# youtalk/opencv-ar

Measured on AMD Instinct MI355X. Metric: frames/sec at 1920x1080, 16 markers/frame; 1/2/4/8 MI355X, higher is better.
Workload: dtype u8

## Files before the change

opencv-ar_amd/csrc/follow.hip:

```cpp
#include "kernels.h"
#include "trace_core.h"

namespace ocvar {

__device__ __forceinline__ int ticket_lane() {
    int l = (int)(threadIdx.x & 63);
    asm volatile("" : "+v"(l));
    return l;
}
__device__ __forceinline__ int uni(int v) { return __builtin_amdgcn_readfirstlane(v); }
__device__ __forceinline__ unsigned uni(unsigned v) { return (unsigned)__builtin_amdgcn_readfirstlane((int)v); }
__device__ __forceinline__ unsigned long long uni(unsigned long long v) {
    return ((unsigned long long)uni((unsigned)(v >> 32)) << 32) | uni((unsigned)v);
}
__device__ __forceinline__ double uni(double v) { return __longlong_as_double((long long)uni((unsigned long long)__double_as_longlong(v))); }

#ifdef OCVAR_PROF
#define PROF_NOW() __builtin_readcyclecounter()
#define PROF_DECL() unsigned long long prof_acc[16] = {0, 0, 0, 0, 0, 0, 0, 0, 0, 0, 0, 0, 0, 0, 0, 0}
#define PROF_ADD(slot, v) do { prof_acc[slot] += (unsigned long long)(v); } while (0)
#define PROF_FLUSH(base) do { if ((threadIdx.x & 63) == 0) for (int i_ = 0; i_ < 16; i_++) if (i_ != 7) atomicAdd(reinterpret_cast<unsigned long long*>(ws.counters + CNT_PROF) + (base) + i_, prof_acc[i_]); } while (0)
#else
#define PROF_NOW() 0ull
#define PROF_DECL() do { } while (0)
#define PROF_ADD(slot, v) do { (void)(v); } while (0)
#define PROF_FLUSH(base) do { } while (0)
#endif

constexpr int FW = 1;
constexpr int FOLLOW_THREADS = 64 * FW;

struct PlaneRef {
    const uint8_t* nbr;
    int ns, sh, img_w, img_h, plane;
};

template <bool CROP>
__device__ __forceinline__ PlaneRef plane_of(const Workspace& ws, int roi) {
    PlaneRef p;
    if (CROP) {
        const Roi r = ws.rois_crop[roi];
        p.ns = r.ns; p.sh = r.sh; p.img_w = r.w; p.img_h = r.h;
        p.nbr = ws.nbr_crop + r.nbr_off;
    } else {
        p.ns = ws.ns; p.sh = ws.sh; p.img_w = ws.W; p.img_h = ws.H;
        p.nbr = ws.nbr_frame + (size_t)roi * nbr_plane_bytes(ws.ns, ws.sh);
    }
    p.plane = p.ns * p.sh;
    return p;
}

template <bool CROP>
__device__ __forceinline__ void emit_quad(const Workspace& ws, const StartCand c, const int* dst);

template <bool CROP>
__device__ __forceinline__ void approximate_and_emit(const Workspace& ws, const StartCand c, const PlaneRef& pl, const int* pts,
                                                     int npts, double perimeter, DpSlice* stack, bool emit = true) {
    int dst[2 * (DP_MAX_OUT + 1)];
    const int m = approx_poly_dp(pts, npts, perimeter * 0.02, dst, stack);
    if (m != 4 || !quad_filter(dst, pl.img_w, pl.img_h)) return;
    if (emit) emit_quad<CROP>(ws, c, dst);
}

template <bool CROP>
__device__ __forceinline__ void emit_quad(const Workspace& ws, const StartCand c, const int* dst) {
    QuadRec q;
    q.roi = c.roi;
    q.start = c.pos;
    for (int k = 0; k < 8; k++) q.pt[k] = dst[k];
    if (CROP) {
        const int slot = atomicAdd(ws.counters + CNT_CROP_QUADS, 1);
        if (slot >= ws.cap_crop_quads) {
            atomicOr(ws.counters + CNT_ERR, ERR_QUAD_OVERFLOW);
            return;
        }
        ws.quads_crop[slot] = q;
        atomicMin(ws.best_crop + c.roi, ((unsigned long long)(unsigned)c.pos << 32) | (unsigned)slot);
    } else {
        const int slot = atomicAdd(ws.n_quads_frame + c.roi, 1);
        if (slot >= ws.maxq) {
            atomicOr(ws.counters + CNT_ERR, ERR_QUAD_OVERFLOW);
            return;
        }
        ws.quads_frame[(size_t)c.roi * ws.maxq + slot] = q;
    }
}

template <int CTRL, int ROWS = 0xf>
__device__ __forceinline__ unsigned dpp_self(unsigned v) {
    return (unsigned)__builtin_amdgcn_update_dpp((int)v, (int)v, CTRL, ROWS, 0xf, false);
}
template <int CTRL, int ROWS = 0xf>
__device__ __forceinline__ unsigned dpp_zero(unsigned v) {
    return (unsigned)__builtin_amdgcn_update_dpp(0, (int)v, CTRL, ROWS, 0xf, false);
}
#define OCVAR_WAVE_LADDER(STEP) \
    STEP(0xB1, 0xf) STEP(0x4E, 0xf) STEP(0x141, 0xf) STEP(0x140, 0xf) STEP(0x142, 0xa) STEP(0x143, 0xc)

__device__ __forceinline__ unsigned wave_max_u32(unsigned v) {
#define STEP(C, R) { const unsigned o = dpp_self<C, R>(v); v = o > v ? o : v; }
    OCVAR_WAVE_LADDER(STEP)
#undef STEP
    return (unsigned)__builtin_amdgcn_readlane((int)v, 63);
}
__device__ __forceinline__ unsigned long long wave_max_u64(unsigned long long v) {
#define STEP(C, R) { const unsigned long long o = ((unsigned long long)dpp_self<C, R>((unsigned)(v >> 32)) << 32) | dpp_self<C, R>((unsigned)v); v = o > v ? o : v; }
    OCVAR_WAVE_LADDER(STEP)
#undef STEP
    return ((unsigned long long)(unsigned)__builtin_amdgcn_readlane((int)(unsigned)(v >> 32), 63) << 32) |
           (unsigned)__builtin_amdgcn_readlane((int)(unsigned)v, 63);
}
typedef unsigned short us2v __attribute__((ext_vector_type(2)));
__device__ __forceinline__ unsigned pk_min(unsigned a, unsigned b) { return __builtin_bit_cast(unsigned, __builtin_elementwise_min(__builtin_bit_cast(us2v, a), __builtin_bit_cast(us2v, b))); }
__device__ __forceinline__ unsigned pk_max(unsigned a, unsigned b) { return __builtin_bit_cast(unsigned, __builtin_elementwise_max(__builtin_bit_cast(us2v, a), __builtin_bit_cast(us2v, b))); }
__device__ __forceinline__ unsigned wave_pk_min(unsigned v) {
#define STEP(C, R) v = pk_min(v, dpp_self<C, R>(v));
    OCVAR_WAVE_LADDER(STEP)
#undef STEP
    return (unsigned)__builtin_amdgcn_readlane((int)v, 63);
}
__device__ __forceinline__ unsigned wave_pk_max(unsigned v) {
#define STEP(C, R) v = pk_max(v, dpp_self<C, R>(v));
    OCVAR_WAVE_LADDER(STEP)
#undef STEP
    return (unsigned)__builtin_amdgcn_readlane((int)v, 63);
}
__device__ __forceinline__ double wave_sum_f64(double v) {
#define STEP(C, R) { const unsigned long long b = (unsigned long long)__double_as_longlong(v); \
                     v += __longlong_as_double((long long)(((unsigned long long)dpp_zero<C, R>((unsigned)(b >> 32)) << 32) | dpp_zero<C, R>((unsigned)b))); }
    OCVAR_WAVE_LADDER(STEP)
#undef STEP
    const unsigned long long b = (unsigned long long)__double_as_longlong(v);
    return __longlong_as_double((long long)(((unsigned long long)(unsigned)__builtin_amdgcn_readlane((int)(unsigned)(b >> 32), 63) << 32) |
                                            (unsigned)__builtin_amdgcn_readlane((int)(unsigned)b, 63)));
}

__device__ __forceinline__ int px_of(unsigned p) { return (int)(p & 0xffffu); }
__device__ __forceinline__ int py_of(unsigned p) { return (int)(p >> 16); }

constexpr int LDS_PTS = SLAB_PTS;
constexpr int DP_DST = 2 * (DP_MAX_OUT + 1);

struct WaveScratch {
    DpSlice stack[DP_STACK];
    int dst[DP_DST];
};

template <bool K32>
__device__ __forceinline__ int wave_approx_dp(const unsigned* src, int count, double parameter, int* dst, DpSlice* stack) {
    const int lane = threadIdx.x & 63;
    float eps = (float)parameter;
    eps *= eps;
    int top = 0, new_count = 0;
    DpSlice slice = {0, 0}, right = {0, 0};
    int sx = 0, sy = 0;
    bool le_eps = false;
    int pos = 0;
    for (int it = 0; it < 3; it++) {
        pos = (pos + right.start) % count;
        const unsigned sp = uni(src[pos]);
        sx = px_of(sp);
        sy = py_of(sp);
        int max_dist = 0;
        if (K32) {
            unsigned best = 0;
            for (int j = 1 + lane; j < count; j += 64) {
                int q = pos + j;
// ... 88 lines not shown
        }
        if (le_eps) {
            if (new_count >= DP_MAX_OUT) return DP_MAX_OUT + 1;
            dst[2 * new_count] = sx;
            dst[2 * new_count + 1] = sy;
            new_count++;
        } else {
            right.end = slice.end;
            slice.end = right.start;
            if (new_count + top + 2 > DP_MAX_OUT) return DP_MAX_OUT + 1;
            if (lane == 0) {
                stack[top] = right;
                stack[top + 1] = slice;
            }
            top += 2;
        }
    }
    __builtin_amdgcn_fence(__ATOMIC_ACQ_REL, "workgroup");
    const int n = new_count;
    int r = n - 1;
    sx = dst[2 * r];
    sy = dst[2 * r + 1];
    if (++r >= n) r = 0;
    int wpos = r;
    int px = dst[2 * r], py = dst[2 * r + 1];
    if (++r >= n) r = 0;
    for (int i = 0; i < n && new_count > 2; i++) {
        const int ex = dst[2 * r], ey = dst[2 * r + 1];
        if (++r >= n) r = 0;
        const int dx = ex - sx, dy = ey - sy;
        int dist = (px - sx) * dy - (py - sy) * dx;
        dist = dist < 0 ? -dist : dist;
        if ((double)dist * dist <= 0.5 * eps * (dx * dx + dy * dy) && dx != 0 && dy != 0) {
            new_count--;
            dst[2 * wpos] = sx = ex;
            dst[2 * wpos + 1] = sy = ey;
            if (++wpos >= n) wpos = 0;
            px = dst[2 * r];
            py = dst[2 * r + 1];
            if (++r >= n) r = 0;
            i++;
            continue;
        }
        dst[2 * wpos] = sx = px;
        dst[2 * wpos + 1] = sy = py;
        if (++wpos >= n) wpos = 0;
        px = ex;
        py = ey;
    }
    __builtin_amdgcn_fence(__ATOMIC_ACQ_REL, "workgroup");
    return new_count;
}

template <bool CROP, bool STAGE>
__device__ __forceinline__ bool wave_finish_packed(const Workspace& ws, const StartCand c, const PlaneRef& pl, const unsigned* gsrc, int npts,
                                                   unsigned* lpts, WaveScratch* sc) {
    const int lane = threadIdx.x & 63;
    if (npts < 4) return false;
    unsigned lo = 0xffffffffu, hi = 0u;
    if (STAGE) {
        unsigned v[LDS_PTS / 64];
#pragma unroll
        for (int k = 0; k < LDS_PTS / 64; k++) {
            const int i = lane + 64 * k;
            v[k] = i < npts ? gsrc[i] : 0u;
        }
#pragma unroll
        for (int k = 0; k < LDS_PTS / 64; k++) {
            const int i = lane + 64 * k;
            if (i < npts) {
                lpts[i] = v[k];
                lo = pk_min(lo, v[k]);
                hi = pk_max(hi, v[k]);
            }
        }
    } else {
        for (int i = lane; i < npts; i += 64) {
            const unsigned p = gsrc[i];
            lo = pk_min(lo, p);
            hi = pk_max(hi, p);
        }
    }
    lo = wave_pk_min(lo);
    hi = wave_pk_max(hi);
    const int bw = px_of(hi) - px_of(lo), bh = py_of(hi) - py_of(lo);
    if (!((long long)bw * bh > 500)) return false;
    __builtin_amdgcn_fence(__ATOMIC_ACQ_REL, "workgroup");
    const unsigned* src = STAGE ? lpts : gsrc;
    double per = 0.0;
    for (int i = lane; i < npts; i += 64) {
        const unsigned p = src[i], q = src[i == 0 ? npts - 1 : i - 1];
        const float dx = (float)px_of(p) - (float)px_of(q), dy = (float)py_of(p) - (float)py_of(q);
        per += (double)sqrt_rn(dx * dx + dy * dy);
    }
    per = wave_sum_f64(per);
#ifdef OCVAR_PROF
    if (lane == 0) atomicAdd(reinterpret_cast<unsigned long long*>(ws.counters + CNT_PROF) + (CROP ? 16 : 0) + 7, 1ull);
#endif
    const bool k32 = npts <= 1024 && (long long)bw * bw + (long long)bh * bh < (1ll << 21);
    const int m = k32 ? wave_approx_dp<true>(src, npts, per * 0.02, sc->dst, sc->stack) : wave_approx_dp<false>(src, npts, per * 0.02, sc->dst, sc->stack);
    if (m != 4) return false;
    int q[8];
#pragma unroll
    for (int k = 0; k < 8; k++) q[k] = uni(sc->dst[k]);
    if (!quad_filter(q, pl.img_w, pl.img_h)) return false;
    if (lane == 0) emit_quad<CROP>(ws, c, q);
    return true;
}

template <bool CROP>
__device__ __forceinline__ int follow_short(const Workspace& ws, const StartCand c) {
    const int BUDGET = SHORT_STEPS;
    const PlaneRef pl = plane_of<CROP>(ws, c.roi);
    if (c.pos <= 0 || c.pos >= pl.plane) return false;
    {
        if (earlier_start_behind(pl.nbr, pl.ns, pl.plane, c.pos, c.is_hole, BACK_STEPS)) return 0;
        if (CROP) {
            const int x = c.pos % pl.ns, y = c.pos / pl.ns;
            return (x == 1 || y == 1) ? 3 : 1;
        }
        const LeanTrace lt = trace_flat(pl.nbr, pl.ns, pl.plane, c.pos, c.is_hole, nullptr, 0, BUDGET);
        if (lt.status == TRACE_OVERRUN) return lt.npts <= 2 ? 2 : 1;
        if (lt.status != TRACE_OK || lt.npts < 4) return 0;
        return 1;
    }
    return 0;
}

template <bool CROP>
__device__ int follow_overflow(const Workspace& ws, const StartCand c, const PlaneRef& pl) {
    const TraceStats st = trace_border<false, false>(pl.nbr, pl.ns, pl.plane, c.pos, c.is_hole, nullptr, 0, ws.mid_steps);
    if (st.status == TRACE_OVERRUN) return 1;
    if (!worth_approximating(st)) return 0;
    const int need = 2 * st.npts + 2 * (st.npts + 2);
    const long long off = atomicAdd(reinterpret_cast<unsigned long long*>(ws.counters + CNT_POOL_INTS), (unsigned long long)need);
    if (off + need > ws.cap_pool_ints) {
        atomicOr(ws.counters + CNT_ERR, ERR_POOL_OVERFLOW);
        return 0;
    }
    int* pts = ws.pool + off;
    trace_border<true, false>(pl.nbr, pl.ns, pl.plane, c.pos, c.is_hole, pts, st.npts, ws.mid_steps);
    approximate_and_emit<CROP>(ws, c, pl, pts, st.npts, st.perimeter, reinterpret_cast<DpSlice*>(pts + 2 * st.npts));
    return 0;
}

constexpr int T1_TICKET = 512;
constexpr int T1_OUT = 128;

template <bool CROP>
__global__ __launch_bounds__(FOLLOW_THREADS) void follow_kernel(Workspace ws) {
    const StartCand* cands = CROP ? ws.cands_crop : ws.cands_frame;
    int n = ws.counters[CROP ? CNT_CROP_CANDS : CNT_FRAME_CANDS];
    const int cap = CROP ? ws.cap_crop_cands : ws.cap_frame_cands;
    if (n > cap) n = cap;
    int* ticket = ws.counters + (CROP ? CNT_TICKET_C : CNT_TICKET_F);
    const int lane = threadIdx.x & 63;
    const int wave = uni((int)(threadIdx.x >> 6));
    const unsigned long long below = (1ull << lane) - 1ull;
    __shared__ StartCand wqueue[FW][128];
// ... 129 lines not shown
    const unsigned dx = (unsigned)(step_dx((int)e) + 1), dy = (unsigned)(step_dy((int)e) + 1);
    const unsigned pw = ((12u - from) & 7u) < t, pe = ((8u - from) & 7u) < t;
    return dx | (dy << 16) | (((e + 5u) & 7u) << 5) | (e << 10) | (pe << 30) | (pw << 31);
}

struct LeanWalk {
    unsigned xy;
    unsigned m;
    unsigned from;
    unsigned pe;
    unsigned xy0, xy1;
    unsigned cxy;
    int npts, step, status;
};

__device__ __forceinline__ void lean_begin(LeanWalk& w, const uint8_t* nbr, int ns, int cpos, int is_hole) {
    const int i0 = cpos - is_hole;
    const int x = i0 % ns, y = i0 / ns;
    w.xy = w.xy0 = (unsigned)x | ((unsigned)y << 16);
    w.cxy = w.xy0 + (unsigned)is_hole;
    w.npts = 0;
    w.step = 0;
    w.status = -1;
    w.xy1 = 0;
    w.pe = 0;
    w.from = 0;
    w.m = nbr_of(nbr, x, y, ns);
    if (w.m == 0) {
        w.status = TRACE_SINGLE;
        w.npts = 1;
        return;
    }
    const int s = first_cw(w.m, (is_hole ? 0 : 4) - 1);
    w.xy1 = w.xy0 + (unsigned)(step_dx(s) + 65536 * step_dy(s));
    w.pe = (unsigned)(s ^ 4) << 10;
    w.from = (unsigned)(s + 1) & 7u;
}

template <class Park>
__device__ __forceinline__ void lean_step(LeanWalk& w, const unsigned* tab, const uint8_t* base, unsigned nt, unsigned last, Park&& park) {
    const unsigned mm = __builtin_amdgcn_perm(w.m, w.m, 0u);
    const unsigned t = (unsigned)__builtin_ctz(__builtin_amdgcn_alignbit(mm, mm, w.from));
    const unsigned ent = tab[(t << 3) + w.from];
    const int d = (int)(w.xy - w.cxy);
    const unsigned nf = ((ent << 1) & (unsigned)(d + 1)) | (ent & (unsigned)d);
    const unsigned nxy = w.xy + (ent & LW_DELTA) - 0x10001u;
    const bool closes = (nxy == w.xy0) & (w.xy == w.xy1);
    const unsigned e = ent & LW_EXIT;
    const bool emit = e != w.pe;
    unsigned off = nbr_win_off_xy(nxy, nt);
    off = off < last ? off : last;
    const unsigned* win = reinterpret_cast<const unsigned*>(base + off);
    const unsigned m4 = nbr_mask9(win[0], win[1], win[2], nxy & 15u);
    park(w.xy);
    w.npts += emit ? 1 : 0;
    w.status = (int)nf < 0 ? (int)TRACE_NOT_FIRST : closes ? (int)TRACE_OK : m4 == 0u ? (int)TRACE_OVERRUN : -1;
    w.step += 1;
    w.xy = nxy;
    w.pe = e;
    w.from = (ent >> 5) & 7u;
    w.m = m4;
}

constexpr int MID_BLOCK = 32;
constexpr int POINT_ROW = MID_BLOCK + 1;
constexpr int FLUSH_W = MID_BLOCK <= 16 ? 16 : 32;
static_assert(FLUSH_W >= MID_BLOCK && 64 % FLUSH_W == 0, "a group of lanes covers a whole row of parked points");

template <bool CROP>
__global__ __launch_bounds__(FOLLOW_THREADS) void follow_mid_kernel(Workspace ws, int phase) {
    __shared__ WaveScratch scratch[FW];
    __shared__ unsigned parked[FW][64 * POINT_ROW];
    __shared__ unsigned step_tab[64];
    if (threadIdx.x < 64u) step_tab[threadIdx.x] = lean_table_entry(threadIdx.x);
    __syncthreads();
    const StartCand* cands = CROP ? ws.mid_crop : ws.mid_frame;
    StartCand* longs = CROP ? ws.long_crop : ws.long_frame;
    int n = ws.counters[CROP ? CNT_MID_C : CNT_MID_F];
    if (n > ws.cap_long) n = ws.cap_long;
    int n_first = (CROP && phase != 2) ? ws.counters[CNT_MID_C_FIRST] : 0;
    if (n_first > ws.cap_long) n_first = ws.cap_long;
    n += n_first;
    int* ticket = ws.counters + (CROP ? (phase == 2 ? CNT_TICKET_MC2 : CNT_TICKET_MC) : CNT_TICKET_MF);
    int* n_long = ws.counters + (CROP ? CNT_LONG_C : CNT_LONG_F);
    const int lane = threadIdx.x & 63;
    const int wave = uni((int)(threadIdx.x >> 6));
    const unsigned long long below = (1ull << lane) - 1ull;
    unsigned* wave_slabs = reinterpret_cast<unsigned*>(ws.slab) + ((size_t)blockIdx.x * blockDim.x + uni((int)(threadIdx.x & ~63u))) * SLAB_STRIDE;
    static_assert(64 * POINT_ROW >= LDS_PTS, "the staging area of the approximation aliases the (flushed) point rows");
    unsigned* my_row = parked[wave] + lane * POINT_ROW;
    const unsigned* wave_rows = parked[wave];
    int flushed = 0;
    const int budget = ws.mid_steps;
    bool have = false;
    bool more = true;
    StartCand c;
    c.roi = 0; c.pos = 0; c.is_hole = 0;
    PlaneRef pl = plane_of<CROP>(ws, 0);
    LeanWalk w;
    w.xy = w.m = w.from = w.pe = w.xy0 = w.xy1 = w.cxy = 0u;
    w.npts = w.step = 0;
    w.status = TRACE_NOT_FIRST;
    unsigned pl_nt = 1u, pl_last = 0u;
    long long guard = ((long long)n + 64) * (budget / MID_BLOCK + 5) + 64;
    PROF_DECL();
    for (;;) {
        if (--guard < 0) {
            if (lane == 0) atomicOr(ws.counters + CNT_ERR, ERR_TICKET_RUNAWAY);
            break;
        }
        const unsigned long long pt0 = PROF_NOW();
        for (int tries = 0; tries < (CROP ? 4 : 1); tries++) {
            const unsigned long long idle = __ballot(!have);
            if (!(more && idle)) break;
            if (tries > 0) --guard;
            const int cnt = __popcll(idle);
            int base = 0;
            if (ticket_lane() == 0) base = atomicAdd(ticket, cnt);
            base = uni(base);
            if (base + cnt >= n) more = false;
            if (!have) {
                const int idx = base + __popcll(idle & below);
                if (idx < n) {
                    c = (CROP && idx < n_first) ? ws.mid_first_crop[idx] : cands[idx - n_first];
                    bool take = true;
                    if (CROP) {
                        const int earliest = ws.crop_min_rest[c.roi];
                        const bool beaten = (unsigned)(ws.best_crop[c.roi] >> 32) < (unsigned)c.pos;
                        if (phase == 1) take = idx < n_first || c.pos == earliest;
                        else if (phase == 2) take = c.pos != earliest && !beaten;
                        else take = !beaten;
                    }
                    pl = plane_of<CROP>(ws, c.roi);
                    if (take && c.pos > 0 && c.pos < pl.plane) {
                        lean_begin(w, pl.nbr, pl.ns, c.pos, c.is_hole);
                        pl_nt = (unsigned)(pl.ns >> 4);
                        pl_last = (unsigned)nbr_plane_bytes(pl.ns, pl.sh) - 12u;
                        have = true;
                        flushed = 0;
                    }
                }
            }
        }
        if (__ballot(have) == 0) break;
        const unsigned long long pt1 = PROF_NOW();
        PROF_ADD(0, pt1 - pt0);
        for (int k = 0; k < MID_BLOCK; k++) {
            const bool running = have && w.status < 0;
            if (__ballot(running) == 0) break;
            PROF_ADD(4, 1);
            PROF_ADD(5, __popcll(__ballot(running)));
            if (running)
                lean_step(w, step_tab, pl.nbr, pl_nt, pl_last, [&](unsigned xy) {
                    const int slot = w.npts - flushed;
                    my_row[slot < MID_BLOCK ? slot : MID_BLOCK] = xy;
                });
        }
        if (have && w.status < 0 && w.step >= budget) w.status = TRACE_OVERRUN;
        const unsigned long long pt2 = PROF_NOW();
        PROF_ADD(1, pt2 - pt1);
        {
            const int stored = w.npts < SLAB_PTS ? w.npts : SLAB_PTS;
            const int pend = have ? stored - flushed : 0;
            unsigned long long fm = __ballot(pend > 0);
            if (fm) __builtin_amdgcn_fence(__ATOMIC_ACQ_REL, "workgroup");
            const int grp = lane / FLUSH_W, k = lane % FLUSH_W;
            while (fm) {
                int L = 0, cnt = 0, off = 0;
#pragma unroll
                for (int g = 0; g < 64 / FLUSH_W; g++) {
                    const int Lg = fm ? __ffsll((long long)fm) - 1 : 0;
                    const int cg = fm ? __builtin_amdgcn_readlane(pend, Lg) : 0;
                    const int og = __builtin_amdgcn_readlane(flushed, Lg);
                    fm &= fm - 1;
                    L = grp == g ? Lg : L;
                    cnt = grp == g ? cg : cnt;
                    off = grp == g ? og : off;
                }
                if (k < cnt) wave_slabs[(size_t)L * SLAB_STRIDE + off + k] = wave_rows[L * POINT_ROW + k];
            }
            flushed += pend;
        }
        const unsigned long long pt3 = PROF_NOW();
        PROF_ADD(2, pt3 - pt2);
        int route = 0, slab_npts = 0;
#ifdef OCVAR_PROF
        {
            const bool done = have && w.status >= 0;
            for (int st_ = 0; st_ < 3; st_++) {
                const int want = st_ == 0 ? (int)TRACE_NOT_FIRST : st_ == 1 ? (int)TRACE_OK : (int)TRACE_OVERRUN;
                const bool mine = done && w.status == want;
                PROF_ADD(9 + 2 * st_, __popcll(__ballot(mine)));
                unsigned steps_ = mine ? (unsigned)w.step : 0u;
                for (int o_ = 32; o_ > 0; o_ >>= 1) steps_ += (unsigned)__shfl_xor((int)steps_, o_, 64);
                PROF_ADD(8 + 2 * st_, steps_);
            }
            bool useless = false;
            if (CROP && done && w.status == TRACE_OK) useless = (unsigned)(ws.best_crop[c.roi] >> 32) < (unsigned)c.pos;
            unsigned us_ = useless ? (unsigned)w.step : 0u;
            for (int o_ = 32; o_ > 0; o_ >>= 1) us_ += (unsigned)__shfl_xor((int)us_, o_, 64);
            PROF_ADD(14, us_);
            PROF_ADD(15, __popcll(__ballot(done && w.status == TRACE_OK && w.npts < 4)));
        }
#endif
        if (have && w.status >= 0) {
            if (w.status == TRACE_OVERRUN) route = 1;
            else if (w.status == TRACE_OK && w.npts >= 4) {
                if (w.npts <= SLAB_PTS) {
                    route = 3;
                    slab_npts = w.npts;
                } else {
                    route = follow_overflow<CROP>(ws, c, pl);
                }
            }
            have = false;
        }
        unsigned long long todo = __ballot(route == 3);
        unsigned my_best = 0xffffffffu;
        if (CROP && route == 3) my_best = (unsigned)(ws.best_crop[c.roi] >> 32);
        if (todo) __builtin_amdgcn_fence(__ATOMIC_ACQ_REL, "workgroup");
        while (todo) {
            const int L = __ffsll((long long)todo) - 1;
            todo &= todo - 1;
            StartCand cl;
            cl.roi = __builtin_amdgcn_readlane(c.roi, L);
            cl.pos = __builtin_amdgcn_readlane(c.pos, L);
            cl.is_hole = __builtin_amdgcn_readlane(c.is_hole, L);
            const int nl = __builtin_amdgcn_readlane(slab_npts, L);
            const unsigned* sl = wave_slabs + (size_t)L * SLAB_STRIDE;
            PlaneRef pll = pl;
            pll.img_w = __builtin_amdgcn_readlane(pl.img_w, L);
            pll.img_h = __builtin_amdgcn_readlane(pl.img_h, L);
            const bool beaten = CROP && (unsigned)__builtin_amdgcn_readlane((int)my_best, L) < (unsigned)cl.pos;
            if (!beaten) wave_finish_packed<CROP, true>(ws, cl, pll, sl, nl, parked[wave], &scratch[wave]);
            PROF_ADD(6, 1);
        }
        PROF_ADD(3, PROF_NOW() - pt3);
        const unsigned long long mask = __ballot(route == 1);
        if (mask) {
            int qbase = 0;
            const int leader = __ffsll((long long)mask) - 1;
            if (lane == leader) qbase = atomicAdd(n_long, __popcll(mask));
            qbase = __builtin_amdgcn_readlane(qbase, leader);
            if (route == 1) {
                const int slot = qbase + __popcll(mask & below);
                if (slot < ws.cap_long) longs[slot] = c;
                else atomicOr(ws.counters + CNT_ERR, ERR_CAND_OVERFLOW);
            }
        }
    }
    PROF_FLUSH(CROP ? 16 : 0);
}

constexpr int TILE_SLOTS = TILE_H + 2;
struct TileCache {
    unsigned* lds;
    const uint8_t* nbr;
    int ns, sh;
    int tx0, ty0;
};

__device__ __forceinline__ void tile_load(TileCache& t, int x, int y, int bx = 0, int by = 0) {
    const int lane = threadIdx.x & 63;
    t.tx0 = (x + 20 * bx - TILE_W / 2 + 8) & ~15;
    t.ty0 = (int)div14((unsigned)(y + 24 * by - 28 + 4 * NBR_TILE_H)) * NBR_TILE_H - 4 * NBR_TILE_H;
    const int tx = (t.tx0 >> 4), ty = t.ty0 / NBR_TILE_H, nty = (t.sh + NBR_TILE_H - 1) / NBR_TILE_H;
    constexpr int NQ = TILE_TX * TILE_TY * 4;
    static_assert(NQ > 64 && NQ <= 128, "two quarter tiles per lane at most");
    uint4 v[2];
#pragma unroll
    for (int h = 0; h < 2; h++) {
        const int q = lane + 64 * h, i = (q >> 2) % TILE_TX, j = (q >> 2) / TILE_TX;
        v[h] = make_uint4(0u, 0u, 0u, 0u);
        if (q < NQ && tx + i >= 0 && (tx + i) * 16 < t.ns && ty + j >= 0 && ty + j < nty)
            v[h] = *reinterpret_cast<const uint4*>(t.nbr + nbr_tile_off((unsigned)(tx + i), (unsigned)(ty + j), t.ns) + 16 * (q & 3));
    }
#pragma unroll
    for (int h = 0; h < 2; h++) {
        const int q = lane + 64 * h, i = (q >> 2) % TILE_TX, j = (q >> 2) / TILE_TX;
        if (q < NQ) {
            unsigned* d = t.lds + i * TILE_SLOTS + NBR_TILE_H * j + 4 * (q & 3);
            d[0] = v[h].x; d[1] = v[h].y; d[2] = v[h].z; d[3] = v[h].w;
        }
    }
    __builtin_amdgcn_fence(__ATOMIC_ACQ_REL, "workgroup");
}

__device__ __forceinline__ unsigned tile_mask(const TileCache& t, int lx, int ly) {
// ... 89 lines not shown
                    if (step >= max_steps) {
                        r.status = TRACE_OVERRUN;
                        bad = true;
                        break;
                    }
                    if (k == 64) continue;
                    if ((close_mask >> k) & 1ull) {
                        closed = true;
                        break;
                    }
                    const unsigned stop_m = (unsigned)__builtin_amdgcn_readlane((int)mq, k);
                    if (stop_m == 256u) {
                        if ((unsigned)(x + ddx) >= (unsigned)ns || (unsigned)(y + ddy) >= (unsigned)t.sh) {
                            r.status = TRACE_OVERRUN;
                            bad = true;
                            break;
                        }
                        tile_load(t, x + ddx, y + ddy, ddx, ddy);
                        continue;
                    }
                    x += ddx;
                    y += ddy;
                    step++;
                    m4 = stop_m;
                    break;
                }
                if (bad || closed) break;
                if (m4 == 0) {
                    r.status = TRACE_OVERRUN;
                    break;
                }
                straight = 0;
            }
        } else {
            straight = 0;
        }
        m = m4;
        s = e ^ 4;
    }
    if (r.status == TRACE_OK) {
        const int stored = r.npts < max_pts ? r.npts : max_pts;
        const int rem = stored & 63;
        if (lane < rem) out1[stored - rem + lane] = hp;
    }
    r.steps = step;
    return r;
}

template <bool CROP>
__global__ __launch_bounds__(FOLLOW_THREADS) void follow_long_kernel(Workspace ws) {
    __shared__ unsigned tiles[FW][TILE_TX * TILE_SLOTS];
    __shared__ WaveScratch scratch[FW];
    __shared__ unsigned staged[FW][LDS_PTS];
    const StartCand* longs = CROP ? ws.long_crop : ws.long_frame;
    int n = ws.counters[CROP ? CNT_LONG_C : CNT_LONG_F];
    if (n > ws.cap_long) n = ws.cap_long;
    int* ticket = ws.counters + (CROP ? CNT_TICKET_LC : CNT_TICKET_LF);
    const int lane = threadIdx.x & 63;
    const int wave = uni((int)(threadIdx.x >> 6));
    int* slab = ws.slab3 + ((size_t)blockIdx.x * FW + wave) * SLAB3_STRIDE;
    for (int guard = n + 2;; guard--) {
        if (guard < 0) {
            if (lane == 0) atomicOr(ws.counters + CNT_ERR, ERR_TICKET_RUNAWAY);
            break;
        }
        int idx = 0;
        if (ticket_lane() == 0) idx = atomicAdd(ticket, 1);
        idx = uni(idx);
        if (idx >= n) break;
        StartCand c = longs[idx];
        c.roi = uni(c.roi);
        c.pos = uni(c.pos);
        c.is_hole = uni(c.is_hole);
        const PlaneRef pl = plane_of<CROP>(ws, c.roi);
        const bool beaten = CROP && uni((unsigned)(ws.best_crop[c.roi] >> 32)) < (unsigned)c.pos;
        TileCache t;
        t.lds = tiles[wave];
        t.nbr = pl.nbr;
        t.ns = uni(pl.ns);
        t.sh = uni(pl.sh);
        t.tx0 = t.ty0 = -(1 << 28);
        LeanTrace lt;
        lt.status = TRACE_NOT_FIRST;
        lt.npts = 0;
        lt.steps = 0;
        if (!beaten) lt = trace_lean_tiled(t, c.pos, c.is_hole, slab, SLAB3_PTS, 4 * uni(pl.plane) + 16);
        if (lt.status == TRACE_OVERRUN) {
            if (lane == 0) atomicOr(ws.counters + CNT_ERR, ERR_TRACE_OVERRUN);
        } else if (lt.status == TRACE_OK && lt.npts >= 4) {
            if (lt.npts > SLAB3_PTS) {
                const long long need = (long long)lt.npts + 64;
                unsigned long long off = 0;
                if (lane == 0) off = atomicAdd(reinterpret_cast<unsigned long long*>(ws.counters + CNT_POOL_INTS), (unsigned long long)need);
                off = uni(off);
                if ((long long)off + need > ws.cap_pool_ints) {
                    if (lane == 0) atomicOr(ws.counters + CNT_ERR, ERR_POOL_OVERFLOW);
                } else {
                    int* big = ws.pool + off;
                    t.tx0 = t.ty0 = -(1 << 28);
                    const LeanTrace lt2 = trace_lean_tiled(t, c.pos, c.is_hole, big, lt.npts, 4 * uni(pl.plane) + 16);
                    __builtin_amdgcn_fence(__ATOMIC_ACQ_REL, "workgroup");
                    if (lt2.status == TRACE_OK && lt2.npts == lt.npts) {
                        wave_finish_packed<CROP, false>(ws, c, pl, reinterpret_cast<const unsigned*>(big), lt2.npts, staged[wave], &scratch[wave]);
                    } else if (lane == 0) {
                        atomicOr(ws.counters + CNT_ERR, ERR_TRACE_OVERRUN);
                    }
                }
            } else {
                __builtin_amdgcn_fence(__ATOMIC_ACQ_REL, "workgroup");
                if (lt.npts <= LDS_PTS) wave_finish_packed<CROP, true>(ws, c, pl, reinterpret_cast<const unsigned*>(slab), lt.npts, staged[wave], &scratch[wave]);
                else wave_finish_packed<CROP, false>(ws, c, pl, reinterpret_cast<const unsigned*>(slab), lt.npts, staged[wave], &scratch[wave]);
            }
        }
    }
}

__device__ __forceinline__ void setup_crop(const Workspace& ws, int f, int i, const float* sq) {
    int quad[8];
    for (int k = 0; k < 8; k++) quad[k] = (int)sq[k];
    int x0, y0, cw, ch, roi_index = -1;
    crop_rect(quad, ws.W, ws.H, &x0, &y0, &cw, &ch);
    const int sw = cw & ~1, sh = ch & ~1, ns = (sw + 15) & ~15;
    if (sw >= 2 && sh >= 2) {
        const int r = atomicAdd(ws.counters + CNT_CROP_ROIS, 1);
        const long long plane = nbr_plane_bytes(ns, sh);
        const long long off = (long long)atomicAdd(ws.crop_pixels, (unsigned long long)plane);
        const int ntx = (sw + MARCH_STRIP - 1) / MARCH_STRIP, nty = (sh + MARCH_CROP_ROWS - 1) / MARCH_CROP_ROWS;
        if (r >= ws.cap_crop_rois || off + plane > ws.cap_crop_pixels) {
            atomicOr(ws.counters + CNT_ERR, ERR_CROP_OVERFLOW);
        } else {
            const int tbase = atomicAdd(ws.counters + CNT_CROP_TILES, ntx * nty);
            if (tbase + ntx * nty > ws.cap_crop_tiles) {
                atomicOr(ws.counters + CNT_ERR, ERR_TILE_OVERFLOW);
            } else {
                Roi roi;
                roi.frame = f; roi.x0 = x0; roi.y0 = y0; roi.w = cw; roi.h = ch; roi.sw = sw; roi.sh = sh; roi.ns = ns;
                roi.owner = i; roi.nbr_off = off;
                ws.rois_crop[r] = roi;
                ws.best_crop[r] = ~0ull;
                ws.crop_min_rest[r] = 0x7fffffff;
                ws.ring_crop[r] = 0;
                for (int t = 0; t < ntx * nty; t++) {
                    TileDesc td;
                    td.roi = r; td.x0 = t % ntx; td.y0 = (t / ntx) * MARCH_CROP_ROWS;
                    ws.tiles_crop[tbase + t] = td;
                }
                roi_index = r;
            }
        }
    }
    ws.crop_of[(size_t)f * ws.maxq + i] = roi_index;
}

__global__ __launch_bounds__(256) void order_and_crops_kernel(Workspace ws) {
    extern __shared__ int order_lds[];
    int* s_start = order_lds;
    float (*s_sq)[8] = reinterpret_cast<float (*)[8]>(order_lds + ws.maxq);
    __shared__ int s_n;
    const int f = blockIdx.x;
    const int tid = threadIdx.x;
    int n = ws.n_quads_frame[f];
    if (n > ws.maxq) n = ws.maxq;
    const QuadRec* q = ws.quads_frame + (size_t)f * ws.maxq;
    for (int i = tid; i < n; i += blockDim.x) s_start[i] = q[i].start;
// ... 204 lines not shown
```

opencv-ar_amd/csrc/trace_core.h:

```cpp
#pragma once
#include "hd.h"
#include <math.h>

namespace ocvar {

OCVAR_HD float sqrt_rn(float v) {
#if defined(__HIP_DEVICE_COMPILE__)
    return __fsqrt_rn(v);
#else
    return sqrtf(v);
#endif
}

OCVAR_HD int first_ccw(unsigned m, int from) {
    from &= 7;
    unsigned r = ((m >> from) | (m << (8 - from))) & 0xFFu;
    return (from + __builtin_ctz(r)) & 7;
}
OCVAR_HD int first_cw(unsigned m, int from) {
    from &= 7;
    unsigned r = ((m << (7 - from)) | (m >> (from + 1))) & 0xFFu;
    return (from - (__builtin_clz(r) - 24)) & 7;
}

// ... 249 lines not shown
    w.prev_s = w.s ^ 4;
}

template <bool BUDGET = true, class Store>
OCVAR_HD void flat_step_t(FlatWalk& w, const uint8_t* nbr, int ns, int plane, int cpos, int max_steps, Store&& store) {
    const int from = (w.s + 1) & 7;
    const int t = __builtin_ctz(((w.m * 0x101u) >> from) & 0xffu);
    const int e = (from + t) & 7;
    const unsigned passed = ((((1u << t) - 1u) * 0x101u) << from) >> 8;
    const bool budget = BUDGET & (w.step >= max_steps);
    const unsigned early = (((unsigned)(w.idx - cpos) >> 31) << 4) | ((unsigned)(w.idx + 1 - cpos) >> 31);
    const bool nf = !budget & ((passed & early) != 0u);
    const int dx = step_dx(e), dy = step_dy(e);
    const int nidx = w.idx + mul_small(dy, ns) + dx;
    const bool closes = !budget & !nf & (nidx == w.i0) & (w.idx == w.i1);
    const bool oob = (unsigned)nidx >= (unsigned)plane;
    const bool emit = !budget & (e != w.prev_s);
    const int lx = w.x + dx, ly = w.y + dy;
    const bool off_plane = oob | ((unsigned)lx >= (unsigned)ns);
    const unsigned m4 = nbr_at(nbr, off_plane ? 0 : lx, off_plane ? 0 : ly, ns);
    store(emit, w.x, w.y);
    w.npts += emit ? 1 : 0;
    w.status = budget ? (int)TRACE_OVERRUN : nf ? (int)TRACE_NOT_FIRST : closes ? (int)TRACE_OK : (oob | (m4 == 0u)) ? (int)TRACE_OVERRUN : -1;
    w.step += w.status < 0 ? 1 : 0;
    w.x = lx;
    w.y = ly;
    w.idx = nidx;
    w.prev_s = e;
    w.m = m4;
    w.s = e ^ 4;
}

OCVAR_HD void flat_step(FlatWalk& w, const uint8_t* nbr, int ns, int plane, int cpos, int* out, int max_pts, int max_steps) {
    flat_step_t(w, nbr, ns, plane, cpos, max_steps, [&](bool emit, int x, int y) {
        if (max_pts > 0) {
            const int slot = (emit && w.npts < max_pts) ? w.npts : max_pts;
            out[2 * slot] = x;
            out[2 * slot + 1] = y;
        }
    });
}

OCVAR_HD LeanTrace trace_flat(const uint8_t* nbr, int ns, int plane, int cpos, int is_hole, int* out, int max_pts, int max_steps) {
    FlatWalk w;
    flat_begin(w, nbr, ns, cpos, is_hole);
    while (w.status < 0) flat_step(w, nbr, ns, plane, cpos, out, max_pts, max_steps);
    LeanTrace r;
    r.status = w.status;
    r.npts = w.npts;
    r.steps = w.step;
    return r;
}

OCVAR_HD TraceStats stats_of_points(const int* pts, int n) {
    TraceStats st;
    st.status = TRACE_OK;
    st.npts = n;
    st.steps = 0;
    st.minx = st.miny = 0x7fffffff;
    st.maxx = st.maxy = -0x7fffffff;
    st.perimeter = 0.0;
    int px = pts[2 * (n - 1)], py = pts[2 * (n - 1) + 1];
    for (int i0 = 0; i0 < n; i0 += 8) {
        int xs[8], ys[8];
#pragma unroll
        for (int k = 0; k < 8; k++) {
            const int q = i0 + k < n ? i0 + k : n - 1;
            xs[k] = pts[2 * q];
            ys[k] = pts[2 * q + 1];
        }
#pragma unroll
        for (int k = 0; k < 8; k++) {
            if (i0 + k >= n) break;
            const int x = xs[k], y = ys[k];
            st.minx = x < st.minx ? x : st.minx;
            st.maxx = x > st.maxx ? x : st.maxx;
            st.miny = y < st.miny ? y : st.miny;
            st.maxy = y > st.maxy ? y : st.maxy;
            if (n > 1) {
                const float dx = (float)x - (float)px, dy = (float)y - (float)py;
                st.perimeter += (double)sqrt_rn(dx * dx + dy * dy);
            }
            px = x;
            py = y;
        }
    }
    return st;
}

OCVAR_HD bool earlier_start_behind(const uint8_t* nbr, int sw, int plane, int cpos, int is_hole, int max_back) {
    const int i0 = cpos - is_hole;
    int x = i0 % sw, y = i0 / sw;
    unsigned m = nbr_at(nbr, x, y, sw);
    if (m == 0) return false;
    const int b0 = first_cw(m, (is_hole ? 0 : 4) - 1);
    int q = i0 + dir_dy(b0) * sw + dir_dx(b0);
    x += dir_dx(b0);
    y += dir_dy(b0);
    int s = (b0 + 4) & 7;
    for (int k = 0; k < max_back; k++) {
        if ((unsigned)q >= (unsigned)plane) return false;
        m = nbr_at(nbr, x, y, sw);
        if (m == 0) return false;
        const int b = first_cw(m, s - 1);
        if (q == i0 && b == b0) return false;
        const int examined = (s - (b + 1)) & 7;
// ... 230 lines not shown
```

Before: 251,700.

## Accumulate contour bbox and perimeter during walk; prefetch next slab into registers

```diff
diff --git a/opencv-ar_amd/csrc/follow.hip b/opencv-ar_amd/csrc/follow.hip
--- a/opencv-ar_amd/csrc/follow.hip
+++ b/opencv-ar_amd/csrc/follow.hip
@@ -16,11 +16,24 @@
 __device__ __forceinline__ double uni(double v) { return __longlong_as_double((long long)uni((unsigned long long)__double_as_longlong(v))); }
 
 #ifdef OCVAR_PROF
+#if OCVAR_PROF >= 2
+#define PROF2_NOW() __builtin_readcyclecounter()
+#define PROF2_ADD(slot, v) do { prof_acc[slot] += (unsigned long long)(v); } while (0)
+#else
+#define PROF2_NOW() 0ull
+#define PROF2_ADD(slot, v) do { (void)(v); } while (0)
+#endif
+#define PROF_PARAM , unsigned long long* prof_acc
+#define PROF_PASS , prof_acc
 #define PROF_NOW() __builtin_readcyclecounter()
 #define PROF_DECL() unsigned long long prof_acc[16] = {0, 0, 0, 0, 0, 0, 0, 0, 0, 0, 0, 0, 0, 0, 0, 0}
 #define PROF_ADD(slot, v) do { prof_acc[slot] += (unsigned long long)(v); } while (0)
 #define PROF_FLUSH(base) do { if ((threadIdx.x & 63) == 0) for (int i_ = 0; i_ < 16; i_++) if (i_ != 7) atomicAdd(reinterpret_cast<unsigned long long*>(ws.counters + CNT_PROF) + (base) + i_, prof_acc[i_]); } while (0)
 #else
+#define PROF2_NOW() 0ull
+#define PROF2_ADD(slot, v) do { (void)(v); } while (0)
+#define PROF_PARAM
+#define PROF_PASS
 #define PROF_NOW() 0ull
 #define PROF_DECL() do { } while (0)
 #define PROF_ADD(slot, v) do { (void)(v); } while (0)
@@ -110,9 +123,8 @@
     return ((unsigned long long)(unsigned)__builtin_amdgcn_readlane((int)(unsigned)(v >> 32), 63) << 32) |
            (unsigned)__builtin_amdgcn_readlane((int)(unsigned)v, 63);
 }
-typedef unsigned short us2v __attribute__((ext_vector_type(2)));
-__device__ __forceinline__ unsigned pk_min(unsigned a, unsigned b) { return __builtin_bit_cast(unsigned, __builtin_elementwise_min(__builtin_bit_cast(us2v, a), __builtin_bit_cast(us2v, b))); }
-__device__ __forceinline__ unsigned pk_max(unsigned a, unsigned b) { return __builtin_bit_cast(unsigned, __builtin_elementwise_max(__builtin_bit_cast(us2v, a), __builtin_bit_cast(us2v, b))); }
+__device__ __forceinline__ unsigned pk_min(unsigned a, unsigned b) { return pk_min_u16(a, b); }
+__device__ __forceinline__ unsigned pk_max(unsigned a, unsigned b) { return pk_max_u16(a, b); }
 __device__ __forceinline__ unsigned wave_pk_min(unsigned v) {
 #define STEP(C, R) v = pk_min(v, dpp_self<C, R>(v));
     OCVAR_WAVE_LADDER(STEP)
@@ -307,28 +319,49 @@
     return new_count;
 }
 
+template <int R>
+__device__ __forceinline__ void stage_load(const unsigned* gsrc, int npts, unsigned (&v)[R]) {
+    const int lane = threadIdx.x & 63;
+#pragma unroll
+    for (int k = 0; k < R; k++) {
+        const int i = lane + 64 * k;
+        v[k] = i < npts ? gsrc[i] : 0u;
+    }
+}
+template <int R>
+__device__ __forceinline__ void stage_store(const unsigned (&v)[R], int npts, unsigned* lpts, unsigned& lo, unsigned& hi) {
+    const int lane = threadIdx.x & 63;
+#pragma unroll
+    for (int k = 0; k < R; k++) {
+        const int i = lane + 64 * k;
+        if (i < npts) {
+            lpts[i] = v[k];
+            lo = pk_min(lo, v[k]);
+            hi = pk_max(hi, v[k]);
+        }
+    }
+}
+
+struct LaneStats {
+    unsigned lo, hi;
+    double per;
+};
+
 template <bool CROP, bool STAGE>
 __device__ __forceinline__ bool wave_finish_packed(const Workspace& ws, const StartCand c, const PlaneRef& pl, const unsigned* gsrc, int npts,
-                                                   unsigned* lpts, WaveScratch* sc) {
+                                                   unsigned* lpts, WaveScratch* sc PROF_PARAM, const LaneStats* ls = nullptr) {
     const int lane = threadIdx.x & 63;
     if (npts < 4) return false;
+    const unsigned long long ft0 = PROF2_NOW();
     unsigned lo = 0xffffffffu, hi = 0u;
-    if (STAGE) {
+    const bool lane_stats = STAGE && ls != nullptr;
+    if (lane_stats) {
+        lo = ls->lo;
+        hi = ls->hi;
+    } else if (STAGE) {
         unsigned v[LDS_PTS / 64];
-#pragma unroll
-        for (int k = 0; k < LDS_PTS / 64; k++) {
-            const int i = lane + 64 * k;
-            v[k] = i < npts ? gsrc[i] : 0u;
-        }
-#pragma unroll
-        for (int k = 0; k < LDS_PTS / 64; k++) {
-            const int i = lane + 64 * k;
-            if (i < npts) {
-                lpts[i] = v[k];
-                lo = pk_min(lo, v[k]);
-                hi = pk_max(hi, v[k]);
-            }
-        }
+        stage_load(gsrc, npts, v);
+        stage_store(v, npts, lpts, lo, hi);
     } else {
         for (int i = lane; i < npts; i += 64) {
             const unsigned p = gsrc[i];
@@ -336,30 +369,54 @@
             hi = pk_max(hi, p);
         }
     }
-    lo = wave_pk_min(lo);
-    hi = wave_pk_max(hi);
+    const unsigned long long ft1 = PROF2_NOW();
+    PROF2_ADD(8, ft1 - ft0);
+    if (!lane_stats) {
+        lo = wave_pk_min(lo);
+        hi = wave_pk_max(hi);
+    }
     const int bw = px_of(hi) - px_of(lo), bh = py_of(hi) - py_of(lo);
-    if (!((long long)bw * bh > 500)) return false;
+    if (!((long long)bw * bh > 500)) {
+        PROF2_ADD(9, PROF2_NOW() - ft1);
+        PROF2_ADD(12, 1);
+        return false;
+    }
     __builtin_amdgcn_fence(__ATOMIC_ACQ_REL, "workgroup");
     const unsigned* src = STAGE ? lpts : gsrc;
     double per = 0.0;
-    for (int i = lane; i < npts; i += 64) {
-        const unsigned p = src[i], q = src[i == 0 ? npts - 1 : i - 1];
-        const float dx = (float)px_of(p) - (float)px_of(q), dy = (float)py_of(p) - (float)py_of(q);
-        per += (double)sqrt_rn(dx * dx + dy * dy);
-    }
-    per = wave_sum_f64(per);
+    if (lane_stats) {
+        per = ls->per + (double)packed_seg(uni(src[0]), uni(src[npts - 1]));
+    } else {
+        for (int i = lane; i < npts; i += 64) {
+            const unsigned p = src[i], q = src[i == 0 ? npts - 1 : i - 1];
+            per += (double)packed_seg(p, q);
+        }
+        per = wave_sum_f64(per);
+    }
+    const unsigned long long ft2 = PROF2_NOW();
+    PROF2_ADD(9, ft2 - ft1);
 #ifdef OCVAR_PROF
     if (lane == 0) atomicAdd(reinterpret_cast<unsigned long long*>(ws.counters + CNT_PROF) + (CROP ? 16 : 0) + 7, 1ull);
 #endif
     const bool k32 = npts <= 1024 && (long long)bw * bw + (long long)bh * bh < (1ll << 21);
     const int m = k32 ? wave_approx_dp<true>(src, npts, per * 0.02, sc->dst, sc->stack) : wave_approx_dp<false>(src, npts, per * 0.02, sc->dst, sc->stack);
-    if (m != 4) return false;
+    const unsigned long long ft3 = PROF2_NOW();
+    PROF2_ADD(10, ft3 - ft2);
+    if (m != 4) {
+        PROF2_ADD(13, 1);
+        return false;
+    }
     int q[8];
 #pragma unroll
     for (int k = 0; k < 8; k++) q[k] = uni(sc->dst[k]);
-    if (!quad_filter(q, pl.img_w, pl.img_h)) return false;
+    if (!quad_filter(q, pl.img_w, pl.img_h)) {
+        PROF2_ADD(11, PROF2_NOW() - ft3);
+        PROF2_ADD(14, 1);
+        return false;
+    }
     if (lane == 0) emit_quad<CROP>(ws, c, q);
+    PROF2_ADD(11, PROF2_NOW() - ft3);
+    PROF2_ADD(15, 1);
     return true;
 }
 
@@ -595,7 +652,7 @@
     off = off < last ? off : last;
     const unsigned* win = reinterpret_cast<const unsigned*>(base + off);
     const unsigned m4 = nbr_mask9(win[0], win[1], win[2], nxy & 15u);
-    park(w.xy);
+    park(w.xy, emit);
     w.npts += emit ? 1 : 0;
     w.status = (int)nf < 0 ? (int)TRACE_NOT_FIRST : closes ? (int)TRACE_OK : m4 == 0u ? (int)TRACE_OVERRUN : -1;
     w.step += 1;
@@ -645,6 +702,8 @@
     w.npts = w.step = 0;
     w.status = TRACE_NOT_FIRST;
     unsigned pl_nt = 1u, pl_last = 0u;
+    WalkStats wst;
+    walk_stats_begin(wst);
     long long guard = ((long long)n + 64) * (budget / MID_BLOCK + 5) + 64;
     PROF_DECL();
     for (;;) {
@@ -677,6 +736,7 @@
                     pl = plane_of<CROP>(ws, c.roi);
                     if (take && c.pos > 0 && c.pos < pl.plane) {
                         lean_begin(w, pl.nbr, pl.ns, c.pos, c.is_hole);
+                        walk_stats_begin(wst);
                         pl_nt = (unsigned)(pl.ns >> 4);
                         pl_last = (unsigned)nbr_plane_bytes(pl.ns, pl.sh) - 12u;
                         have = true;
@@ -694,9 +754,10 @@
             PROF_ADD(4, 1);
             PROF_ADD(5, __popcll(__ballot(running)));
             if (running)
-                lean_step(w, step_tab, pl.nbr, pl_nt, pl_last, [&](unsigned xy) {
+                lean_step(w, step_tab, pl.nbr, pl_nt, pl_last, [&](unsigned xy, bool emit) {
                     const int slot = w.npts - flushed;
                     my_row[slot < MID_BLOCK ? slot : MID_BLOCK] = xy;
+                    walk_stats_point(wst, emit, w.npts == 0, xy);
                 });
         }
         if (have && w.status < 0 && w.step >= budget) w.status = TRACE_OVERRUN;
@@ -727,7 +788,7 @@
         const unsigned long long pt3 = PROF_NOW();
         PROF_ADD(2, pt3 - pt2);
         int route = 0, slab_npts = 0;
-#ifdef OCVAR_PROF
+#if defined(OCVAR_PROF) && OCVAR_PROF < 2
         {
             const bool done = have && w.status >= 0;
             for (int st_ = 0; st_ < 3; st_++) {
@@ -758,10 +819,17 @@
             }
             have = false;
         }
-        unsigned long long todo = __ballot(route == 3);
-        unsigned my_best = 0xffffffffu;
-        if (CROP && route == 3) my_best = (unsigned)(ws.best_crop[c.roi] >> 32);
+        bool go = route == 3;
+        PROF_ADD(6, __popcll(__ballot(go)));
+        go = go && walk_stats_worth(wst.lo, wst.hi);
+        PROF2_ADD(12, __popcll(__ballot(route == 3 && !go)));
+        if (CROP && go) go = !((unsigned)(ws.best_crop[c.roi] >> 32) < (unsigned)c.pos);
+        unsigned long long todo = __ballot(go);
         if (todo) __builtin_amdgcn_fence(__ATOMIC_ACQ_REL, "workgroup");
+        constexpr int PF_REGS = 4;
+        unsigned pf[PF_REGS] = {};
+        bool prefetched = false;
+        unsigned* lpts = parked[wave];
         while (todo) {
             const int L = __ffsll((long long)todo) - 1;
             todo &= todo - 1;
@@ -774,9 +842,33 @@
             PlaneRef pll = pl;
             pll.img_w = __builtin_amdgcn_readlane(pl.img_w, L);
             pll.img_h = __builtin_amdgcn_readlane(pl.img_h, L);
-            const bool beaten = CROP && (unsigned)__builtin_amdgcn_readlane((int)my_best, L) < (unsigned)cl.pos;
-            if (!beaten) wave_finish_packed<CROP, true>(ws, cl, pll, sl, nl, parked[wave], &scratch[wave]);
-            PROF_ADD(6, 1);
+            LaneStats ls;
+            ls.lo = (unsigned)__builtin_amdgcn_readlane((int)wst.lo, L);
+            ls.hi = (unsigned)__builtin_amdgcn_readlane((int)wst.hi, L);
+            const unsigned long long perb = (unsigned long long)__double_as_longlong(wst.per);
+            ls.per = __longlong_as_double((long long)(((unsigned long long)(unsigned)__builtin_amdgcn_readlane((int)(unsigned)(perb >> 32), L) << 32) |
+                                                      (unsigned)__builtin_amdgcn_readlane((int)(unsigned)perb, L)));
+            const unsigned long long st0 = PROF2_NOW();
+            unsigned box_lo = 0u, box_hi = 0u;
+            if (prefetched) {
+                stage_store(pf, nl, lpts, box_lo, box_hi);
+            } else {
+                unsigned v[LDS_PTS / 64];
+                stage_load(sl, nl, v);
+                stage_store(v, nl, lpts, box_lo, box_hi);
+            }
+            prefetched = false;
+            if (todo) {
+                const int Ln = __ffsll((long long)todo) - 1;
+                const int nn = __builtin_amdgcn_readlane(slab_npts, Ln);
+                if (nn <= 64 * PF_REGS) {
+                    stage_load(wave_slabs + (size_t)Ln * SLAB_STRIDE, nn, pf);
+                    prefetched = true;
+                }
+            }
+            __builtin_amdgcn_fence(__ATOMIC_ACQ_REL, "workgroup");
+            PROF2_ADD(8, PROF2_NOW() - st0);
+            wave_finish_packed<CROP, true>(ws, cl, pll, sl, nl, lpts, &scratch[wave] PROF_PASS, &ls);
         }
         PROF_ADD(3, PROF_NOW() - pt3);
         const unsigned long long mask = __ballot(route == 1);
@@ -972,6 +1064,7 @@
     __shared__ unsigned tiles[FW][TILE_TX * TILE_SLOTS];
     __shared__ WaveScratch scratch[FW];
     __shared__ unsigned staged[FW][LDS_PTS];
+    PROF_DECL();
     const StartCand* longs = CROP ? ws.long_crop : ws.long_frame;
     int n = ws.counters[CROP ? CNT_LONG_C : CNT_LONG_F];
     if (n > ws.cap_long) n = ws.cap_long;
@@ -1021,15 +1114,15 @@
                     const LeanTrace lt2 = trace_lean_tiled(t, c.pos, c.is_hole, big, lt.npts, 4 * uni(pl.plane) + 16);
                     __builtin_amdgcn_fence(__ATOMIC_ACQ_REL, "workgroup");
                     if (lt2.status == TRACE_OK && lt2.npts == lt.npts) {
-                        wave_finish_packed<CROP, false>(ws, c, pl, reinterpret_cast<const unsigned*>(big), lt2.npts, staged[wave], &scratch[wave]);
+                        wave_finish_packed<CROP, false>(ws, c, pl, reinterpret_cast<const unsigned*>(big), lt2.npts, staged[wave], &scratch[wave] PROF_PASS);
                     } else if (lane == 0) {
                         atomicOr(ws.counters + CNT_ERR, ERR_TRACE_OVERRUN);
                     }
                 }
             } else {
                 __builtin_amdgcn_fence(__ATOMIC_ACQ_REL, "workgroup");
-                if (lt.npts <= LDS_PTS) wave_finish_packed<CROP, true>(ws, c, pl, reinterpret_cast<const unsigned*>(slab), lt.npts, staged[wave], &scratch[wave]);
-                else wave_finish_packed<CROP, false>(ws, c, pl, reinterpret_cast<const unsigned*>(slab), lt.npts, staged[wave], &scratch[wave]);
+                if (lt.npts <= LDS_PTS) wave_finish_packed<CROP, true>(ws, c, pl, reinterpret_cast<const unsigned*>(slab), lt.npts, staged[wave], &scratch[wave] PROF_PASS);
+                else wave_finish_packed<CROP, false>(ws, c, pl, reinterpret_cast<const unsigned*>(slab), lt.npts, staged[wave], &scratch[wave] PROF_PASS);
             }
         }
     }
diff --git a/opencv-ar_amd/csrc/trace_core.h b/opencv-ar_amd/csrc/trace_core.h
--- a/opencv-ar_amd/csrc/trace_core.h
+++ b/opencv-ar_amd/csrc/trace_core.h
@@ -325,6 +325,74 @@
     return r;
 }
 
+OCVAR_HD unsigned pk_min_u16(unsigned a, unsigned b) {
+#if defined(__HIP_DEVICE_COMPILE__)
+    typedef unsigned short us2 __attribute__((ext_vector_type(2)));
+    return __builtin_bit_cast(unsigned, __builtin_elementwise_min(__builtin_bit_cast(us2, a), __builtin_bit_cast(us2, b)));
+#else
+    const unsigned al = a & 0xffffu, bl = b & 0xffffu, ah = a >> 16, bh = b >> 16;
+    return (al < bl ? al : bl) | ((ah < bh ? ah : bh) << 16);
+#endif
+}
+OCVAR_HD unsigned pk_max_u16(unsigned a, unsigned b) {
+#if defined(__HIP_DEVICE_COMPILE__)
+    typedef unsigned short us2 __attribute__((ext_vector_type(2)));
+    return __builtin_bit_cast(unsigned, __builtin_elementwise_max(__builtin_bit_cast(us2, a), __builtin_bit_cast(us2, b)));
+#else
+    const unsigned al = a & 0xffffu, bl = b & 0xffffu, ah = a >> 16, bh = b >> 16;
+    return (al > bl ? al : bl) | ((ah > bh ? ah : bh) << 16);
+#endif
+}
+OCVAR_HD float packed_seg(unsigned p, unsigned q) {
+    const float dx = (float)(int)(p & 0xffffu) - (float)(int)(q & 0xffffu), dy = (float)(int)(p >> 16) - (float)(int)(q >> 16);
+    return sqrt_rn(dx * dx + dy * dy);
+}
+
+struct WalkStats {
+    unsigned lo, hi;
+    unsigned last;
+    double per;
+};
+
+OCVAR_HD void walk_stats_begin(WalkStats& s) {
+    s.lo = 0xffffffffu;
+    s.hi = 0u;
+    s.last = 0u;
+    s.per = 0.0;
+}
+OCVAR_HD void walk_stats_point(WalkStats& s, bool emit, bool first, unsigned xy) {
+    const double seg = (double)packed_seg(xy, s.last);
+    s.per += (emit & !first) ? seg : 0.0;
+    s.lo = emit ? pk_min_u16(s.lo, xy) : s.lo;
+    s.hi = emit ? pk_max_u16(s.hi, xy) : s.hi;
+    s.last = emit ? xy : s.last;
+}
+OCVAR_HD double walk_stats_perimeter(const WalkStats& s, unsigned first_pt) { return s.per + (double)packed_seg(first_pt, s.last); }
+OCVAR_HD bool walk_stats_worth(unsigned lo, unsigned hi) {
+    const long long bw = (long long)(hi & 0xffffu) - (long long)(lo & 0xffffu), bh = (long long)(hi >> 16) - (long long)(lo >> 16);
+    return bw * bh > 500;
+}
+
+OCVAR_HD LeanTrace trace_flat_stats(const uint8_t* nbr, int ns, int plane, int cpos, int is_hole, int* out, int max_pts, int max_steps, WalkStats& st) {
+    FlatWalk w;
+    flat_begin(w, nbr, ns, cpos, is_hole);
+    walk_stats_begin(st);
+    while (w.status < 0)
+        flat_step_t(w, nbr, ns, plane, cpos, max_steps, [&](bool emit, int x, int y) {
+            walk_stats_point(st, emit, w.npts == 0, (unsigned)x | ((unsigned)y << 16));
+            if (max_pts > 0) {
+                const int slot = (emit && w.npts < max_pts) ? w.npts : max_pts;
+                out[2 * slot] = x;
+                out[2 * slot + 1] = y;
+            }
+        });
+    LeanTrace r;
+    r.status = w.status;
+    r.npts = w.npts;
+    r.steps = w.step;
+    return r;
+}
+
 OCVAR_HD TraceStats stats_of_points(const int* pts, int n) {
     TraceStats st;
     st.status = TRACE_OK;
```

After: 248,100. 1.4% lower.
